# ifpen/wfcrl-env

Hardware: NVIDIA B200
Metric: Floris env-steps/sec (HornsRev1) (higher is better)
Workload: dtype f32

## Files before the change

### wfcrl_b200/csrc/wf_device.cuh

```cuda
#pragma once
#include "../../include/wfcrl_b200.h"

#include <cuda_runtime.h>
#include <stdint.h>

#define WF_MAX_TURBINES_K 128
#define WF_FIX_REC_HDR 5
#define WF_NP 9

struct WfModel {
    int T, B;
    int max_iter, continuous, multi_agent, shaper, table_len;
    int G;
    float yaw_lo_f, yaw_hi_f, yaw_step_f;
    float rate_f, dt_f;
    int autoreset;
    unsigned long long ar_seed;
    long long ar_offset;
    double ar_ti_lo, ar_ti_hi;
    int vtab_tmajor;
    float amb_eps;
    double load_coef, shaper_reference;
    double rho, ref_rho, shear, D, HH, TSR, pP;
    double alpha, beta, ka, kb, ad, bd, dm;
    double ch_const, ch_ai, ch_init, ch_down;
    double e3_112, e3_13;
    const double* layout_c;
    int n_layouts;
    int sample_layouts;
    const double* tab_ws;
    const double* tab_ct;
    const double* tab_pw;
    const double* layout_x;
    const double* layout_y;
};

__host__ __device__ inline const int* layout_counts(const WfModel& m) { return (const int*)(m.layout_c + 2 * m.n_layouts); }

struct WfState {
    double* yaw;
    float* acc;
    float* acc_prev;
    int* num_iter;
    int* num_moves;
    int* nonfinite;
    int* episode;
    uint8_t* amb;
    double* ep_return;
    int* ep_len;
    double* fin_sum;
    double* fin_sumsq;
    int* fin_n;
    long long* fin_len;
    uint8_t* reset_mask;
    int* fix_list;
    int* fix_count;
    double* ws;
    double* wd;
    double* ws_norm;
    double* shaper_ref;
    double* ti_amb;
    double* xs;
    double* ys;
    double* xi;
    double* yi;
    int* order;
    double* cs;
    float2* xhl;
    float2* yhl;
    uchar4* idx;
    double* vtab;
    uint8_t* vtab_ok;
    uint8_t* tab_lo;
    uint8_t* tab_glo;
    double2* vwg;
    int* layout_id;
    int* turbine_count;
};

template <typename R> struct WfFastConstT {
    R ratio[3];
    R mean_ratio;
    R nu4[3];
    R zz[6][3];
    R zz2[6][3];
    R ez[6][3];
    R cblk[48];
    R a_top, a_bot, a_core;
    R inv_ss_den;
    R cv[3][9], cw[3][9];
    R sv[3];
    R D, inv_D, eps2, inv_eps2, inv_2pi;
    R c_top, c_bot, c_wr;
    R alpha4, beta2, ka, kb, ad, bd, dm03, e3_112, e3_13;
    R near_c;
    R d2_8;
    R ch_const, ch_ai, ch_init, ch_down;
    R pP3, rho_fac, ref_rho, two_D, offj[3], dz2[3];
    R load_coef, shaper_reference;
    int table_len;
    R tab_ws[64], tab_ct[64], tab_pw[64];
    unsigned char coarse[128];
    R coarse_scale;
    int coarse_len;
};
typedef WfFastConstT<float> WfFastConst;
typedef WfFastConstT<double> WfFastConst64;

enum WfMode { WF_MODE_INTERFACE = 0, WF_MODE_ENV = 1, WF_MODE_WARMUP = 2 };

struct WfEvalArgs {
    int K;
    int* fix_list;
    int* fix_count;
    uint8_t* amb;
    double2* vwg;
};

cudaError_t wf_launch_geometry(const WfModel& m, const WfState& s, const uint8_t* d_mask, const double* d_cs_override,
                               cudaStream_t stream, bool autoreset_draw = false);
cudaError_t wf_launch_step_basic(int precision, int mode, const WfModel& m, const WfState& s, const uint8_t* d_mask,
                                 const float* d_action, const double* d_yaw_cmd, const WfStepOut& out,
                                 int env_begin, int env_count, cudaStream_t stream);
cudaError_t wf_launch_vortex_table(const WfModel& m, const WfFastConst64& fc, const WfState& s, const uint8_t* d_mask,
                                   cudaStream_t stream);
cudaError_t wf_launch_set_wind(const WfModel& m, const WfState& s, const uint8_t* d_mask, const double* d_ws,
                               const double* d_wd, cudaStream_t stream);
cudaError_t wf_launch_sample_reset(const WfModel& m, const WfState& s, const uint8_t* d_mask, unsigned long long seed,
                                   long long env_id_offset, double ti_lo, double ti_hi, double* d_ws, double* d_wd,
                                   cudaStream_t stream);
cudaError_t wf_launch_reset_state(const WfModel& m, const WfState& s, const uint8_t* d_mask, const double* d_ws,
                                  const double* d_wd, cudaStream_t stream);
cudaError_t wf_step_basic_attributes(int precision, cudaFuncAttributes* attr, int* ctas_per_sm, int threads);
cudaError_t wf_configure_fast_kernels();
cudaError_t wf_configure_fast64_kernels();
cudaError_t wf_launch_step_fast(int mode, bool baked, const WfModel& m, const WfFastConst& fc, const WfState& s,
                                const uint8_t* d_mask, const float* d_action, const double* d_yaw_cmd,
                                const WfStepOut& out, int env_begin, int env_count, cudaStream_t stream);
cudaError_t wf_launch_fixup64(int mode, bool use_vtab, const WfModel& m, const WfFastConst64& fc, const WfState& s,
                              const WfStepOut& out, int env_count, float* d_rec, int rec_cap, cudaStream_t stream);
cudaError_t wf_step_fast_attributes(bool baked, const WfModel& m, cudaFuncAttributes* attr, int* ctas_per_sm, int* threads,
                                    int* smem);
cudaError_t wf_launch_step_fast64(int mode, bool use_vtab, const WfModel& m, const WfFastConst64& fc, const WfState& s,
                                  const uint8_t* d_mask, const float* d_action, const double* d_yaw_cmd,
                                  const WfStepOut& out, int env_begin, int env_count, cudaStream_t stream);
cudaError_t wf_step_fast64_attributes(const WfModel& m, const WfState& s, cudaFuncAttributes* attr, int* ctas_per_sm, int* threads,
                                      int* smem);
cudaError_t wf_launch_eval_fast(bool baked, const WfModel& m, const WfFastConst& fc, const WfState& s, const WfEvalArgs& ev,
                                const double* d_yaw, void* d_power, cudaStream_t stream);
cudaError_t wf_launch_eval_fast64(bool use_vtab, const WfModel& m, const WfFastConst64& fc, const WfState& s,
                                  const WfEvalArgs& ev, const double* d_yaw, void* d_power, cudaStream_t stream);
cudaError_t wf_launch_eval_fixup64(bool use_vtab, const WfModel& m, const WfFastConst64& fc, const WfState& s,
                                   const WfEvalArgs& ev, const double* d_yaw, void* d_power, cudaStream_t stream);
bool wf_fast64_gathers(const WfModel& m, const WfState& s);
```

### wfcrl_b200/csrc/wf_fast.cu

```cuda
#include "wf_device.cuh"
#include "wf_reset_device.cuh"
#include "wf_fast_baked.inc"

namespace {

#define KC(name) (BAKED ? WfBaked::name : fc.name)


constexpr float kLog2e = 1.4426950408889634f;
constexpr float kLn2 = 0.6931471805599453f;
constexpr float kDeg = 57.29577951308232f;
constexpr float kRad = 0.017453292519943295f;
constexpr float kNumEpsF = 0.001f;
constexpr int kTurbPerPass = 10;
constexpr int kMaxEvt = 8;

__device__ __forceinline__ float frcp(float x) { float y; asm("rcp.approx.ftz.f32 %0, %1;" : "=f"(y) : "f"(x)); return y; }
__device__ __forceinline__ float fsqrt(float x) { float y; asm("sqrt.approx.ftz.f32 %0, %1;" : "=f"(y) : "f"(x)); return y; }
__device__ __forceinline__ float fex2(float x) { float y; asm("ex2.approx.ftz.f32 %0, %1;" : "=f"(y) : "f"(x)); return y; }
__device__ __forceinline__ float flg2(float x) { float y; asm("lg2.approx.ftz.f32 %0, %1;" : "=f"(y) : "f"(x)); return y; }
__device__ __forceinline__ float fclamp(float x, float lo, float hi) { return fminf(fmaxf(x, lo), hi); }

__device__ __forceinline__ float interp_f(const WfFastConst& fc, const float* __restrict__ fp, float x, float left,
                                          float right) {
    const int n = fc.table_len;
    const float x0 = fc.tab_ws[0], xn = fc.tab_ws[n - 1];
    if (x < x0) return left;
    if (x > xn) return right;
    int bkt = (int)((x - x0) * fc.coarse_scale);
    bkt = min(bkt, fc.coarse_len - 1);
    int idx = fc.coarse[bkt];
    while (idx + 1 < n - 1 && fc.tab_ws[idx + 1] <= x) ++idx;
    const float xa = fc.tab_ws[idx], fa = fp[idx];
    const float slope = (fp[idx + 1] - fa) * frcp(fc.tab_ws[idx + 1] - xa);
    return fmaf(slope, x - xa, fa);
}

struct SmemView {
    float* wsq;
    float2* vw;
    float2 *xhl, *yhl;
    float *tia;
    float *cyaw, *syaw, *yawr;
    float *tifin;
    float *ynew;
    uchar4* idx;
    unsigned char* ordr;
    unsigned char* queue;
    float4* cblk;
    float* evt_ta;
    uchar2* evt_tj;
};

__host__ __device__ inline size_t fast_smem_bytes(int T) {
    size_t n = 12 * 16;
    n += (size_t)kMaxEvt * 4 + 16;
    n += (size_t)3 * 9 * T * 4;
    n += (size_t)2 * T * 8;
    n += (size_t)3 * T * 4;
    n += (size_t)5 * T * 4;
    n += (size_t)T * 4;
    n += (size_t)((T + 15) / 16 * 16);
    n += (size_t)((T + 15) / 16 * 16);
    return (n + 15) / 16 * 16;
}

__device__ __forceinline__ SmemView carve(unsigned char* base, int T) {
    SmemView s;
    s.cblk = (float4*)base;
    s.evt_ta = (float*)(base + 12 * 16);
    s.evt_tj = (uchar2*)(base + 12 * 16 + kMaxEvt * 4);
    float2* f2 = (float2*)(base + 12 * 16 + kMaxEvt * 4 + 16);
    s.xhl = f2;
    s.yhl = f2 + T;
    s.vw = f2 + 2 * T;
    float* f = (float*)(f2 + 2 * T + 9 * T);
    s.wsq = f; f += 9 * T;
    s.tia = f; f += 3 * T;
    s.cyaw = f; f += T;
    s.syaw = f; f += T;
    s.yawr = f; f += T;
    s.tifin = f; f += T;
    s.ynew = f; f += T;
    s.idx = (uchar4*)f; f += T;
    s.ordr = (unsigned char*)f;
    s.queue = s.ordr + (T + 15) / 16 * 16;
    return s;
}

struct wf_true_tag { static constexpr bool value = true; };
struct wf_false_tag { static constexpr bool value = false; };

template <bool BAKED, bool EVAL = false>
__global__ void __launch_bounds__(32, BAKED ? 16 : 12)
wf_step_fast_kernel(const int mode_, const int env_begin, const WfModel m, const __grid_constant__ WfFastConst fc,
                    const WfState s, const uint8_t* __restrict__ mask, const float* __restrict__ action,
                    const double* __restrict__ yaw_cmd, const WfStepOut out, const WfEvalArgs ev) {
    int b;
    if constexpr (EVAL) b = blockIdx.x / ev.K; else b = blockIdx.x + env_begin;
    const int mode = EVAL ? (int)WF_MODE_INTERFACE : mode_;
    if (mask && !mask[b]) return;
    const int T = m.T;
    const int lane = threadIdx.x;
    const size_t row = (size_t)b * T;
    const size_t orow = EVAL ? (size_t)blockIdx.x * T : row;
    extern __shared__ __align__(16) unsigned char smem_raw[];
    const SmemView sm = carve(smem_raw, T);
    const int n = s.turbine_count[b];

    int nm = 0;
    if (mode == WF_MODE_ENV) nm = s.num_moves[b] + 1;
    for (int tt = lane; tt < n; tt += 32) {
        float ynew;
        if (mode == WF_MODE_ENV) {
            float a = action[row + tt];
            const float acc = s.acc[row + tt];
            const float acc_c = (m.multi_agent && tt != n - 1) ? s.acc_prev[row + tt] : acc;
            const float frac = __fdiv_rn(__fdiv_rn(__fdiv_rn(acc_c, m.rate_f), (float)nm), m.dt_f);
            if (frac >= 0.1f) a = 0.0f;
            if (m.continuous) a = fminf(fmaxf(a, -m.yaw_step_f), m.yaw_step_f);
            else a = __fmul_rn(__fsub_rn(a, 1.0f), m.yaw_step_f);
            const float y0 = fminf(fmaxf((float)s.yaw[row + tt], m.yaw_lo_f), m.yaw_hi_f);
            ynew = fminf(fmaxf(__fadd_rn(y0, a), m.yaw_lo_f), m.yaw_hi_f);
            s.acc_prev[row + tt] = acc;
            s.acc[row + tt] = __fadd_rn(acc, fabsf(a));
            s.yaw[row + tt] = (double)ynew;
        } else if (mode == WF_MODE_INTERFACE && yaw_cmd) {
            const double y = yaw_cmd[orow + tt];
            if (!EVAL) s.yaw[row + tt] = y;
            ynew = (float)y;
        } else {
            ynew = (float)s.yaw[row + tt];
        }
        sm.ynew[tt] = ynew;
        sm.xhl[tt] = s.xhl[row + tt];
        sm.yhl[tt] = s.yhl[row + tt];
        sm.idx[tt] = s.idx[row + tt];
        sm.ordr[tt] = (unsigned char)s.order[row + tt];
    }
    if (lane < 12) sm.cblk[lane] = make_float4(fc.cblk[4 * lane], fc.cblk[4 * lane + 1], fc.cblk[4 * lane + 2], fc.cblk[4 * lane + 3]);
    for (int q = lane; q < 9 * n; q += 32) { sm.wsq[q] = 0.f; sm.vw[q] = make_float2(0.f, 0.f); }
    for (int q = lane; q < 3 * n; q += 32) sm.tia[q] = 0.f;
    __syncwarp();
    for (int tt = lane; tt < n; tt += 32) {
        const float yr = sm.ynew[sm.ordr[tt]] * kRad;
        float sy, cy;
        sincosf(yr, &sy, &cy);
        sm.yawr[tt] = yr;
        sm.cyaw[tt] = cy;
        sm.syaw[tt] = sy;
    }
    const double ws_d = s.ws[b], wd_d = s.wd[b];
    const float ws = (float)ws_d;
    const float I0 = (float)s.ti_amb[b];
    const float I02 = I0 * I0;
    const float I0p = __powf(I0, fc.ch_init);
    const float U0a = ws * fc.ratio[0], U0b = ws * fc.ratio[1], U0c = ws * fc.ratio[2];
    const float D = KC(D);
    __syncwarp();

    const int g = lane / 3, j = lane - 3 * g;
    const bool lane_ok = lane < 3 * kTurbPerPass;
    const float offj = (j == 0) ? fc.offj[0] : ((j == 1) ? fc.offj[1] : fc.offj[2]);
    const int pl = lane & 15;
    const bool pv = pl < 9;
    const int plc = pv ? pl : 0;
    const float U0p = (plc % 3 == 0) ? U0a : ((plc % 3 == 1) ? U0b : U0c);
    const float cvl0 = fc.cv[0][plc], cvl1 = fc.cv[1][plc], cvl2 = fc.cv[2][plc];
    const float cwl0 = fc.cw[0][plc], cwl1 = fc.cw[1][plc], cwl2 = fc.cw[2][plc];
    const float c_dec = KC(eps2) * KC(inv_2pi);
    const float c_e = -KC(inv_eps2) * kLog2e;
    const float c_ek = -(0.5f * kLog2e) * (BAKED ? WfBaked::dz2_0 : fc.dz2[0]);
    const float eps2 = KC(eps2);
    const bool strict = m.amb_eps > 0.f;
    const float thr_lo = 0.05f * (1.f - m.amb_eps), thr_hi = 0.05f * (1.f + m.amb_eps);
    const double two_D_d = 2.0 * m.D;
    int nevt = 0;
    bool flagged = false;

    for (int i = 0; i < n; ++i) {
        float su3, sv, sw, vq, wwq;
        {
            const float wq = sm.wsq[9 * i + plc];
            const float2 vw0 = sm.vw[9 * i + plc];
            vq = vw0.x;
            wwq = vw0.y;
            const float u = U0p - fsqrt(wq);
            su3 = pv ? u * u * u : 0.f;
            sv = pv ? vq : 0.f;
            sw = pv ? wwq : 0.f;
#pragma unroll
            for (int sft = 8; sft > 0; sft >>= 1) {
                su3 += __shfl_xor_sync(0xffffffffu, su3, sft);
                sv += __shfl_xor_sync(0xffffffffu, sv, sft);
                sw += __shfl_xor_sync(0xffffffffu, sw, sft);
            }
        }
        const float avg = cbrtf(su3 * (1.f / 9.f));
        const float ct_raw = fclamp(interp_f(fc, fc.tab_ct, avg, 0.0001f, 0.9999f), 0.0001f, 0.9999f);
        const float cy = sm.cyaw[i], sy = sm.syaw[i], yr = sm.yawr[i];
        const float ct = ct_raw * cy;
        const float s1c = fsqrt(1.f - ct * cy);
        const float a = 0.5f * frcp(cy) * (1.f - s1c);
        const float Gtop0 = KC(c_top) * ws * ct, Gbot0 = KC(c_bot) * ws * ct;
        const float Gwr = KC(c_wr) * (a - a * a) * avg;
        const float Gt = sy * cy * Gtop0, Gb = -(sy * cy * Gbot0);

        float val = 2.f * (sv * (1.f / 9.f) - Gwr * KC(a_core)) * frcp(Gtop0 * KC(a_top) - Gbot0 * KC(a_bot));
        val = fclamp(val, -1.f, 1.f);
        const float g_rad = -(yr + 0.5f * asinf(val));
        const float cg = __cosf(g_rad);

        const float sq1ct = fsqrt(1.f - ct);
        const float sqcg = fsqrt(1.f - ct * cg);
        const float sz0d = 0.5f * D * fsqrt((1.f + sqcg) * frcp(2.f * (1.f + sq1ct)));
        const float sy0d = sz0d * cg;
        const float C0 = 1.f - sq1ct;
        const float M0 = C0 * (2.f - C0);
        const float E0 = C0 * C0 - KC(e3_112) * C0 + KC(e3_13);
        const float th = KC(dm03) * g_rad * frcp(cg) * (1.f - sqcg);
        const float sM0 = fsqrt(M0);
        const float tan_th = __sinf(th) * frcp(__cosf(th));
        const float Kc = th * E0 * (1.f / 5.2f) * fsqrt(sy0d * sz0d * frcp(M0));
        const float A_ln = (1.6f + sM0) * frcp(1.6f - sM0);
        const float inv_s0d = frcp(sy0d * sz0d);

        for (int e = 0; e < min(nevt, kMaxEvt); ++e) {
            const uchar2 tj = sm.evt_tj[e];
            if ((int)tj.x == i && sm.evt_ta[e] > sm.tia[3 * i + tj.y]) flagged = true;
        }
        const float ta0 = sm.tia[3 * i], ta1 = sm.tia[3 * i + 1], ta2 = sm.tia[3 * i + 2];
        const float tp0 = fsqrt(fmaf(ta0, ta0, I02)), tp1 = fsqrt(fmaf(ta1, ta1, I02)), tp2 = fsqrt(fmaf(ta2, ta2, I02));
        const float tpre = (j == 0) ? tp0 : ((j == 1) ? tp1 : tp2);
        const float beta_term = KC(beta2) * (1.f - sq1ct);
        const float x0d = D * cg * (1.f + sqcg) * frcp(1.4142135623730951f * fmaf(KC(alpha4), tpre, beta_term));
        const float kyd = fmaf(KC(ka), tpre, KC(kb));
        const float inv_x0d = frcp(x0d);
        const float delta0 = tan_th * x0d;
        const float Kck = Kc * frcp(kyd);

        const uchar4 ix = sm.idx[i];
        const bool self_on = (int)ix.x <= i;
        float sumV = sv, sumW = sw;
        if (self_on) {
            sumV += Gt * (BAKED ? WfBaked::sv0 : fc.sv[0]) + Gb * (BAKED ? WfBaked::sv1 : fc.sv[1]) +
                    Gwr * (BAKED ? WfBaked::sv2 : fc.sv[2]);
            const float Vs = Gt * cvl0 + Gb * cvl1 + Gwr * cvl2;
            const float Ws = fmaxf(Gt * cwl0 + Gb * cwl1 + Gwr * cwl2, 0.f);
            float rw = pv ? Ws : 0.f;
#pragma unroll
            for (int sft = 8; sft > 0; sft >>= 1) rw += __shfl_xor_sync(0xffffffffu, rw, sft);
            sumW += rw;
            __syncwarp();
            if (lane < 9) sm.vw[9 * i + lane] = make_float2(vq + Vs, wwq + Ws);
        }
        const float aI = avg * tp0;
        const float kk2 = 3.f * aI * aI;
        const float v_term = sumV * (1.f / 9.f), w_term = sumW * (1.f / 9.f);
        const float k_total = 0.5f * (kk2 + v_term * v_term + w_term * w_term);
        const float I_mix = fsqrt((2.f / 3.f) * k_total) * frcp(avg) - tp0;
        const float tq0 = fmaf(2.f, I_mix, tp0), tq1 = fmaf(2.f, I_mix, tp1), tq2 = fmaf(2.f, I_mix, tp2);
        if (lane == 0) sm.tifin[i] = (tq0 + tq1 + tq2) * (1.f / 3.f);
        const float tpost = (j == 0) ? tq0 : ((j == 1) ? tq1 : tq2);

        const float x0v = D * cy * (1.f + sq1ct) * frcp(1.4142135623730951f * fmaf(KC(alpha4), tpost, beta_term));
        const float kyv = fmaf(KC(ka), tpost, KC(kb));
        const float inv_x0v = frcp(x0v);
        const float sz0v = KC(near_c) * (0.5f / 0.501f);
        const float sy0v = sz0v * cy;
        const float near_s = KC(near_c) * fsqrt(ct);
        const float ctc = ct * cy * KC(d2_8);
        const float watK = KC(ch_const) * __powf(a, KC(ch_ai)) * I0p;

        const int lo = ix.x, near_i = ix.y, gt0_i = ix.z, end15 = ix.w;
        const float2 xi = sm.xhl[i], yi = sm.yhl[i];

        constexpr float kCut = 5.5f;
        const float reach1 = kCut * kyv;
        const float reach0 = fmaf(kCut, fmaxf(near_s, sy0v), fabsf(delta0) + fabsf(Kck) * (flg2(A_ln) * kLn2));

        int qn = 0;
        auto v_pass = [&](auto yawed_tag, const int t0) {
            constexpr bool YAWED = decltype(yawed_tag)::value;
            const int tr = t0 + g;
            const bool active = lane_ok && tr < n && tr != i;
            const int t = min(tr, n - 1);
            const float2 xt = sm.xhl[t], yt = sm.yhl[t];
            const float dx = (xt.x - xi.x) + (xt.y - xi.y);
            const float dyc = ((yt.x - yi.x) + (yt.y - yi.y)) + offj;

            const bool need = active && (t >= near_i) &&
                              (fabsf(dyc) < fmaf(reach1, dx, reach0) + fabsf(fmaf(KC(bd), dx, KC(ad))));
            const unsigned nb = __ballot_sync(0xffffffffu, need);
            const bool leader = (j == 0) && active && (((nb >> (3 * g)) & 7u) != 0u);
            const unsigned lb = __ballot_sync(0xffffffffu, leader);
            if (leader) sm.queue[qn + __popc(lb & ((1u << lane) - 1u))] = (unsigned char)t;
            qn += __popc(lb);

            const float yL = dyc + kNumEpsF;
            const float q = yL * yL;
            const float E = fex2(q * c_e);
            float Vk[3], Wk[3];
#pragma unroll
            for (int k = 0; k < 3; ++k) {
                float4 ca, cb, cc, cd;
                if (BAKED) {
                    ca = make_float4(WfBaked::cblk(16 * k), WfBaked::cblk(16 * k + 1), WfBaked::cblk(16 * k + 2), WfBaked::cblk(16 * k + 3));
                    cb = make_float4(WfBaked::cblk(16 * k + 4), WfBaked::cblk(16 * k + 5), WfBaked::cblk(16 * k + 6), WfBaked::cblk(16 * k + 7));
                    cc = make_float4(WfBaked::cblk(16 * k + 8), WfBaked::cblk(16 * k + 9), WfBaked::cblk(16 * k + 10), WfBaked::cblk(16 * k + 11));
                    cd = make_float4(WfBaked::cblk(16 * k + 12), WfBaked::cblk(16 * k + 13), WfBaked::cblk(16 * k + 14), WfBaked::cblk(16 * k + 15));
                } else {
                    ca = sm.cblk[4 * k]; cb = sm.cblk[4 * k + 1]; cc = sm.cblk[4 * k + 2]; cd = sm.cblk[4 * k + 3];
                }
                const float r4 = q + cb.x, r5 = q + cb.y;
                const float g4 = Gwr * frcp(r4 * r5);
                const float X4 = fmaf(-E, cc.x, 1.f) * r5;
                const float NV4 = fmaf(cd.y, X4, -(cd.z * r4));
                float SV, SW;
                if (YAWED) {
                    const float r0 = q + ca.x, r2 = q + ca.y, r1 = q + ca.z, r3 = q + ca.w;
                    const float g0 = Gt * frcp(r0 * r2), g1 = Gb * frcp(r1 * r3);
                    const float X0 = fmaf(-E, cb.z, 1.f) * r2, X1 = fmaf(-E, cb.w, 1.f) * r3;
                    const float NV0 = fmaf(cc.y, X0, -(cc.z * r0)), NV1 = fmaf(cc.w, X1, -(cd.x * r1));
                    SV = fmaf(g4, NV4, fmaf(g1, NV1, g0 * NV0));
                    SW = fmaf(g4, X4 - r4, fmaf(g1, X1 - r1, g0 * (X0 - r0)));
                } else {
                    SV = g4 * NV4;
                    SW = g4 * (X4 - r4);
                }
                const float dec = c_dec * frcp(fmaf(cd.w, dx, eps2));
                Vk[k] = SV * dec;
                Wk[k] = fmaxf(SW * (-yL * dec), 0.f);
            }
            if (active) {
                const int qb = 9 * t + 3 * j;
#pragma unroll
                for (int k = 0; k < 3; ++k) {
                    const float2 o = sm.vw[qb + k];
                    sm.vw[qb + k] = make_float2(o.x + Vk[k], o.y + Wk[k]);
                }
            }
        };
        if (sy != 0.f) {
#pragma unroll 2
            for (int t0 = lo; t0 < n; t0 += kTurbPerPass) v_pass(wf_true_tag{}, t0);
        } else {
#pragma unroll 2
            for (int t0 = lo; t0 < n; t0 += kTurbPerPass) v_pass(wf_false_tag{}, t0);
        }
        __syncwarp();

#pragma unroll 1
        for (int q0 = 0; q0 < qn; q0 += kTurbPerPass) {
            const int e = q0 + g;
            const bool active = lane_ok && e < qn;
            const int t = sm.queue[min(e, qn - 1)];
            const float2 xt = sm.xhl[t], yt = sm.yhl[t];
            const float dx = (xt.x - xi.x) + (xt.y - xi.y);
            const float dyc = ((yt.x - yi.x) + (yt.y - yi.y)) + offj;
            const float lin = fmaf(KC(bd), dx, KC(ad));

            float defl;
            {
                const float dd = dx - x0d;
                const float sgy = fmaf(kyd, dd, sy0d), sgz = fmaf(kyd, dd, sz0d);
                const float sq = fsqrt(sgy * sgz * inv_s0d);
                const float L = flg2(A_ln * fmaf(1.6f, sq, -sM0) * frcp(fmaf(1.6f, sq, sM0))) * kLn2;
                const float d_far = fmaf(Kck, L, delta0) + lin;
                const float d_near = fmaf(dx * inv_x0d, delta0, lin);
                defl = (dx <= x0d) ? d_near : d_far;
            }
            float base, ek;
            {
                const bool far = dx >= x0v;
                const float dd = dx - x0v;
                const float up = dx * inv_x0v, down = 1.f - up;
                const float sgy = far ? fmaf(kyv, dd, sy0v) : fmaf(down, near_s, up * sy0v);
                const float sgz = far ? fmaf(kyv, dd, sz0v) : fmaf(down, near_s, up * sz0v);
                const float ry = frcp(sgy), rz = frcp(sgz);
                const float dy = (dyc - defl) * ry;
                const float dcl = fclamp(fmaf(-ctc * ry, rz, 1.f), 0.f, 1.f);
                const float C = 1.f - fsqrt(dcl);
                base = C * fex2((-0.5f * kLog2e) * dy * dy);
                ek = fex2(c_ek * rz * rz);
            }
            const float be = base * ek;
            const float dU0 = be * U0a, dU1 = base * U0b, dU2 = be * U0c;
            int c = 0;
            if (active) {
                c = ((dU0 > thr_hi) + (dU1 > thr_hi) + (dU2 > thr_hi)) |
                    (((dU0 > thr_lo) + (dU1 > thr_lo) + (dU2 > thr_lo)) << 8);
                const int qb = 9 * t + 3 * j;
                sm.wsq[qb] = fmaf(dU0, dU0, sm.wsq[qb]);
                sm.wsq[qb + 1] = fmaf(dU1, dU1, sm.wsq[qb + 1]);
                sm.wsq[qb + 2] = fmaf(dU2, dU2, sm.wsq[qb + 2]);
            }
            const int gb = 3 * g;
            const int c_tot = __shfl_sync(0xffffffffu, c, gb & 31) + __shfl_sync(0xffffffffu, c, (gb + 1) & 31) +
                              __shfl_sync(0xffffffffu, c, (gb + 2) & 31);
            const int c_lo = c_tot & 0xff, c_hi = c_tot >> 8;
            bool ambiguous = false;
            float ta_hi = 0.f;
            if (active && c_hi > 0 && t >= gt0_i && t < end15) {
                const float ady = fabsf(dyc);
                bool in_win = ady < KC(two_D);
                if (fabsf(ady - KC(two_D)) < 2e-3f) {
                    const double d = (((double)yt.x - (double)yi.x) + ((double)yt.y - (double)yi.y)) + (double)offj;
                    in_win = fabs(d) < two_D_d;
                    if (strict && fabs(fabs(d) - two_D_d) < 1e-7) flagged = true;
                }
                if (in_win) {
                    const float wat = watK * __powf(dx * KC(inv_D), KC(ch_down));
                    if (c_lo > 0) sm.tia[3 * t + j] = fmaxf(sm.tia[3 * t + j], (float)c_lo * (1.f / 9.f) * wat);
                    ambiguous = c_hi != c_lo;
                    ta_hi = (float)c_hi * (1.f / 9.f) * wat;
                }
            }
            const unsigned ab = __ballot_sync(0xffffffffu, ambiguous);
            if (ab) {
                const int slot = nevt + __popc(ab & ((1u << lane) - 1u));
                if (ambiguous) {
                    if (slot < kMaxEvt) { sm.evt_ta[slot] = ta_hi; sm.evt_tj[slot] = make_uchar2((unsigned char)t, (unsigned char)j); }
                    else flagged = true;
                }
                nevt += __popc(ab);
            }
        }
        __syncwarp();
    }

    const bool env = (mode != WF_MODE_INTERFACE);
    const float wd = (float)wd_d;
    float rsum_p = 0.f, rsum_l = 0.f;
    for (int tt = lane; tt < n; tt += 32) {
        float u[9], vv[9], ww[9];
        float su = 0.f, su3 = 0.f, svv = 0.f, sww = 0.f, sdd = 0.f;
#pragma unroll
        for (int p = 0; p < 9; ++p) {
            const float U0k = (p % 3 == 0) ? U0a : ((p % 3 == 1) ? U0b : U0c);
            u[p] = U0k - fsqrt(sm.wsq[9 * tt + p]);
            const float2 vwp = sm.vw[9 * tt + p];
            vv[p] = vwp.x;
            ww[p] = vwp.y;
            su += u[p];
            su3 = fmaf(u[p] * u[p], u[p], su3);
            svv += vv[p];
            sww += ww[p];
            sdd += atan2f(vv[p], u[p]);
        }
        const float avg = cbrtf(su3 * (1.f / 9.f));
        const float mu = su * (1.f / 9.f), mv = svv * (1.f / 9.f), mw = sww * (1.f / 9.f);
        float qu = 0.f, qv = 0.f, qw = 0.f;
#pragma unroll
        for (int p = 0; p < 9; ++p) {
            qu = fmaf(u[p] - mu, u[p] - mu, qu);
            qv = fmaf(vv[p] - mv, vv[p] - mv, qv);
            qw = fmaf(ww[p] - mw, ww[p] - mw, qw);
        }
        const float veff = fc.rho_fac * avg * __powf(sm.cyaw[tt], fc.pP3);
        const float pw = interp_f(fc, fc.tab_pw, veff, 0.f, 0.f) * fc.ref_rho;
        if (strict) {
            constexpr float kVelEps = 1.2e-5f;
            const float pm = interp_f(fc, fc.tab_pw, veff * (1.f - kVelEps), 0.f, 0.f) * fc.ref_rho;
            const float pp = interp_f(fc, fc.tab_pw, veff * (1.f + kVelEps), 0.f, 0.f) * fc.ref_rho;
            if (fmaxf(fabsf(pp - pw), fabsf(pw - pm)) > 1e-4f * fmaxf(pw, 1.f)) flagged = true;
        }
        float wsl = avg;
        float wdl = wd - kDeg * sdd * (1.f / 9.f);
        float loads[4] = {sm.tifin[tt], fsqrt(qu * (1.f / 9.f)), fsqrt(qv * (1.f / 9.f)), fsqrt(qw * (1.f / 9.f))};
        float p_out;
        if (env) {
            p_out = pw * 1e-6f;
            rsum_p += p_out;
            rsum_l += fabsf(loads[0]) + fabsf(loads[1]) + fabsf(loads[2]) + fabsf(loads[3]);
        } else {
            p_out = pw;
#pragma unroll
            for (int q = 0; q < 4; ++q) loads[q] *= 1e7f;
        }
        const int orig = sm.ordr[tt];
        if (EVAL) {
            sm.tifin[tt] = p_out;
            continue;
        }
        float yv = sm.ynew[orig];
        if (mode == WF_MODE_WARMUP) {
            wsl = fclamp(wsl, 3.f, 28.f);
            wdl = fclamp(wdl, 0.f, 360.f);
            yv = fclamp(yv, m.yaw_lo_f, m.yaw_hi_f);
        }
        const size_t o = row + orig;
        if (out.yaw) ((float*)out.yaw)[o] = yv;
        if (out.wind_speed) ((float*)out.wind_speed)[o] = wsl;
        if (out.wind_direction) ((float*)out.wind_direction)[o] = wdl;
        if (out.power) ((float*)out.power)[o] = p_out;
        if (out.load) ((float4*)out.load)[o] = make_float4(loads[0], loads[1], loads[2], loads[3]);
    }
#pragma unroll
    for (int sft = 16; sft > 0; sft >>= 1) {
        rsum_p += __shfl_xor_sync(0xffffffffu, rsum_p, sft);
        rsum_l += __shfl_xor_sync(0xffffffffu, rsum_l, sft);
    }
    const bool any_flag = __any_sync(0xffffffffu, flagged);
    if constexpr (EVAL) {
        if (lane == 0 && ev.amb) ev.amb[blockIdx.x] = (uint8_t)any_flag;
        if (any_flag && strict) {
            if (lane == 0) ev.fix_list[atomicAdd(&ev.fix_count[0], 1)] = blockIdx.x;
            return;
        }
        float* const pw_out = (float*)out.power + orow;
        for (int tt = lane; tt < n; tt += 32) pw_out[sm.ordr[tt]] = sm.tifin[tt];
        for (int tt = n + lane; tt < T; tt += 32) pw_out[tt] = 0.f;
        return;
    }
    if (lane == 0 && s.amb) s.amb[b] = (uint8_t)any_flag;
    if (any_flag && strict) {
        if (lane == 0) s.fix_list[atomicAdd(&s.fix_count[0], 1)] = b;
        return;
    }
    int it = 0;
    if (lane == 0) {
        it = s.num_iter[b] + 1;
        s.num_iter[b] = it;
        if (out.truncated) out.truncated[b] = (uint8_t)(it == m.max_iter);
        float fw0 = ws, fw1 = wd;
        if (mode == WF_MODE_WARMUP) { fw0 = fclamp(fw0, 3.f, 28.f); fw1 = fclamp(fw1, 0.f, 360.f); }
        if (out.freewind) ((float2*)out.freewind)[b] = make_float2(fw0, fw1);
        if (mode == WF_MODE_ENV) {
            s.num_moves[b] = nm;
            const float wn = (float)s.ws_norm[b];
            const float invT = 1.f / (float)n;
            float reward = rsum_p * 1e3f / (wn * wn * wn) * invT - fc.load_coef * rsum_l * (0.25f * invT);
            if (m.shaper == 1) {
                reward = (reward - fc.shaper_reference) / fc.shaper_reference;
            } else if (m.shaper == 2) {
                const double ref = s.shaper_ref[b];
                const float shaped = (ref == 0.0) ? 0.f : (float)(((double)reward - ref) / ref);
                s.shaper_ref[b] = (double)reward;
                reward = shaped;
            }
            if (!isfinite(reward)) s.nonfinite[b] += 1;
            if (out.reward) ((float*)out.reward)[b] = reward;
            wfreset::episode_account(s, b, (double)reward, it == m.max_iter);
            s.ws_norm[b] = ws_d;
        }
    }
    if (mode == WF_MODE_ENV && m.autoreset && __shfl_sync(0xffffffffu, (int)(it == m.max_iter), 0)) {
        for (int tt = lane; tt < T; tt += 32) { s.yaw[row + tt] = 0.0; s.acc[row + tt] = 0.f; s.acc_prev[row + tt] = 0.f; }
        if (lane == 0) wfreset::autoreset_mark(s, b);
    }
    auto zero_padding = [&](void* p, const int w) {
        if (p)
#pragma unroll 1
            for (int q = n * w + lane; q < T * w; q += 32) ((float*)p)[row * w + q] = 0.f;
    };
    zero_padding(out.yaw, 1);
    zero_padding(out.wind_speed, 1);
    zero_padding(out.wind_direction, 1);
    zero_padding(out.power, 1);
    zero_padding(out.load, 4);
}

}

cudaError_t wf_configure_fast_kernels() {
    for (auto k : {wf_step_fast_kernel<true>, wf_step_fast_kernel<false>, wf_step_fast_kernel<true, true>,
                   wf_step_fast_kernel<false, true>}) {
        cudaError_t e = cudaFuncSetAttribute(k, cudaFuncAttributeMaxDynamicSharedMemorySize, 64 * 1024);
        if (e == cudaSuccess)
            e = cudaFuncSetAttribute(k, cudaFuncAttributePreferredSharedMemoryCarveout, cudaSharedmemCarveoutMaxShared);
        if (e != cudaSuccess) return e;
    }
    return cudaSuccess;
}

template <bool BAKED>
static cudaError_t launch_fast_t(int mode, const WfModel& m, const WfFastConst& fc, const WfState& s,
                                 const uint8_t* d_mask, const float* d_action, const double* d_yaw_cmd,
                                 const WfStepOut& out, int env_begin, int env_count, cudaStream_t stream) {
    wf_step_fast_kernel<BAKED><<<env_count, 32, fast_smem_bytes(m.T), stream>>>(mode, env_begin, m, fc, s, d_mask, d_action,
                                                                               d_yaw_cmd, out, WfEvalArgs{});
    return cudaGetLastError();
}

template <bool BAKED>
static cudaError_t launch_eval_t(const WfModel& m, const WfFastConst& fc, const WfState& s, const WfEvalArgs& ev,
                                 const double* d_yaw, void* d_power, cudaStream_t stream) {
    WfStepOut out = {};
    out.power = d_power;
    wf_step_fast_kernel<BAKED, true><<<(unsigned)m.B * (unsigned)ev.K, 32, fast_smem_bytes(m.T), stream>>>(
        WF_MODE_INTERFACE, 0, m, fc, s, nullptr, nullptr, d_yaw, out, ev);
    return cudaGetLastError();
}

cudaError_t wf_launch_eval_fast(bool baked, const WfModel& m, const WfFastConst& fc, const WfState& s, const WfEvalArgs& ev,
                                const double* d_yaw, void* d_power, cudaStream_t stream) {
    return baked ? launch_eval_t<true>(m, fc, s, ev, d_yaw, d_power, stream)
                 : launch_eval_t<false>(m, fc, s, ev, d_yaw, d_power, stream);
}

cudaError_t wf_launch_step_fast(int mode, bool baked, const WfModel& m, const WfFastConst& fc, const WfState& s,
                                const uint8_t* d_mask, const float* d_action, const double* d_yaw_cmd,
                                const WfStepOut& out, int env_begin, int env_count, cudaStream_t stream) {
    return baked ? launch_fast_t<true>(mode, m, fc, s, d_mask, d_action, d_yaw_cmd, out, env_begin, env_count, stream)
                 : launch_fast_t<false>(mode, m, fc, s, d_mask, d_action, d_yaw_cmd, out, env_begin, env_count, stream);
}

template <bool BAKED>
static cudaError_t attrs_fast_t(const WfModel& m, cudaFuncAttributes* attr, int* ctas_per_sm, int* threads, int* smem) {
    *threads = 32;
    *smem = (int)fast_smem_bytes(m.T);
    cudaError_t e = cudaFuncGetAttributes(attr, wf_step_fast_kernel<BAKED>);
    if (e != cudaSuccess) return e;
    return cudaOccupancyMaxActiveBlocksPerMultiprocessor(ctas_per_sm, wf_step_fast_kernel<BAKED>, 32, *smem);
}

cudaError_t wf_step_fast_attributes(bool baked, const WfModel& m, cudaFuncAttributes* attr, int* ctas_per_sm, int* threads,
                                    int* smem) {
    return baked ? attrs_fast_t<true>(m, attr, ctas_per_sm, threads, smem) : attrs_fast_t<false>(m, attr, ctas_per_sm, threads, smem);
}
```

### wfcrl_b200/csrc/wf_host_const.h

```cpp
#pragma once
#include "../../include/wfcrl_b200.h"
#include "wf_device.cuh"

#include <math.h>
#include <string.h>

static inline void wf_fill_default_config(WfConfig* c) {
    memset(c, 0, sizeof(*c));
    c->precision = WF_PREC_F64;
    c->kernel = WF_KERNEL_BASIC;
    c->continuous_control = 1;
    c->reward_shaper = WF_SHAPER_NONE;
    c->yaw_lo = -40.0; c->yaw_hi = 40.0; c->yaw_step = 5.0;
    c->load_coef = 0.1;
    c->shaper_reference = 0.0;
    c->dt = 60.0;
    c->actuator_rate = 0.3;
    c->air_density = 1.225; c->turbulence_intensity = 0.06; c->wind_shear = 0.12; c->wind_veer = 0.0;
    c->alpha = 0.58; c->beta = 0.077; c->ka = 0.38; c->kb = 0.004; c->ad = 0.0; c->bd = 0.0; c->dm = 1.0;
    c->ch_initial = 0.1; c->ch_constant = 0.5; c->ch_ai = 0.8; c->ch_downstream = -0.32;
    c->turbine_grid_points = 3;
    c->rotor_diameter = 126.0; c->hub_height = 90.0; c->tsr = 8.0; c->pP = 1.88; c->pT = 1.88;
    c->generator_efficiency = 1.0; c->ref_density_cp_ct = 1.225;
    static const double cp[51] = {
        0.0, 0.0, 0.0, 0.178085, 0.289075, 0.349022, 0.384728, 0.406059, 0.420228, 0.428823, 0.433873, 0.436223,
        0.436845, 0.436575, 0.436511, 0.436561, 0.436517, 0.435903, 0.434673, 0.433230, 0.430466, 0.378869, 0.335199,
        0.297991, 0.266092, 0.238588, 0.214748, 0.193981, 0.175808, 0.159835, 0.145741, 0.133256, 0.122157, 0.112257,
        0.103399, 0.095449, 0.088294, 0.081836, 0.075993, 0.070692, 0.065875, 0.061484, 0.057476, 0.053809, 0.050447,
        0.047358, 0.044518, 0.041900, 0.039483, 0.0, 0.0};
    static const double ct[51] = {
        0.0, 0.0, 0.0, 0.99, 0.99, 0.97373036, 0.92826162, 0.89210543, 0.86100905, 0.835423, 0.81237673, 0.79225789,
        0.77584769, 0.7629228, 0.76156073, 0.76261984, 0.76169723, 0.75232027, 0.74026851, 0.72987175, 0.70701647,
        0.54054532, 0.45509459, 0.39343381, 0.34250785, 0.30487242, 0.27164979, 0.24361964, 0.21973831, 0.19918151,
        0.18131868, 0.16537679, 0.15103727, 0.13998636, 0.1289037, 0.11970413, 0.11087113, 0.10339901, 0.09617888,
        0.09009926, 0.08395078, 0.0791188, 0.07448356, 0.07050731, 0.06684119, 0.06345518, 0.06032267, 0.05741999,
        0.05472609, 0.0, 0.0};
    c->table_len = 51;
    c->table_ws[0] = 0.0; c->table_ws[1] = 2.0; c->table_ws[2] = 2.5;
    for (int i = 0; i < 45; ++i) c->table_ws[3 + i] = 3.0 + 0.5 * i;
    c->table_ws[48] = 25.01; c->table_ws[49] = 25.02; c->table_ws[50] = 50.0;
    for (int i = 0; i < 51; ++i) { c->table_cp[i] = cp[i]; c->table_ct[i] = ct[i]; }
    }

template <typename R> static inline void build_fast_const(const WfConfig& c, WfFastConstT<R>* f) {
    memset(f, 0, sizeof(*f));
    const double PI = 3.141592653589793, NUM_EPS = 0.001;
    const double D = c.rotor_diameter, HH = c.hub_height, eps = 0.2 * D, eps2 = eps * eps, off = 0.5 * D / 2;
    double Z[3], ratio[3], rsum = 0.0;
    for (int k = 0; k < 3; ++k) {
        Z[k] = HH + (k - 1) * off;
        ratio[k] = pow(Z[k] / HH, c.wind_shear);
        rsum += ratio[k];
    }
    const double mean_ratio = rsum / 3.0;
    f->mean_ratio = (R)mean_ratio;
    const double zc[6] = {-(HH + D / 2), -(HH - D / 2), (HH + D / 2), (HH - D / 2), -HH, HH};
    double zz[6][3];
    for (int k = 0; k < 3; ++k) {
        f->ratio[k] = (R)ratio[k];
        const double dU = c.wind_shear * pow(1.0 / HH, c.wind_shear) * pow(Z[k], c.wind_shear - 1.0);
        const double lmda = D / 8, kappa = 0.41;
        const double lm = kappa * Z[k] / (1 + kappa * Z[k] / lmda);
        f->nu4[k] = (R)(4 * lm * lm * fabs(dU) / mean_ratio);
        for (int q = 0; q < 6; ++q) {
            zz[q][k] = (Z[k] + zc[q]) + NUM_EPS;
            f->zz[q][k] = (R)zz[q][k];
            f->zz2[q][k] = (R)(zz[q][k] * zz[q][k]);
            f->ez[q][k] = (R)exp(-zz[q][k] * zz[q][k] / eps2);
        }
        f->dz2[k] = (R)(((k - 1) * off) * ((k - 1) * off));
        f->offj[k] = (R)((k - 1) * off);
    }
    for (int k = 0; k < 3; ++k) {
        R* c = f->cblk + 16 * k;
        c[0] = f->zz2[0][k]; c[1] = f->zz2[2][k]; c[2] = f->zz2[1][k]; c[3] = f->zz2[3][k];
        c[4] = f->zz2[4][k]; c[5] = f->zz2[5][k]; c[6] = f->ez[0][k]; c[7] = f->ez[1][k];
        c[8] = f->ez[4][k]; c[9] = f->zz[0][k]; c[10] = f->zz[2][k]; c[11] = f->zz[1][k];
        c[12] = f->zz[3][k]; c[13] = f->zz[4][k]; c[14] = f->zz[5][k]; c[15] = f->nu4[k];
    }
    double a_top = 0, a_bot = 0, a_core = 0, sv[3] = {0, 0, 0};
    for (int p = 0; p < 9; ++p) {
        const int j = p / 3, k = p % 3;
        const double yL = (j - 1) * off + NUM_EPS, q = yL * yL;
        double fq[6];
        for (int v = 0; v < 6; ++v) {
            const double r = q + zz[v][k] * zz[v][k];
            fq[v] = (1 - exp(-r / eps2)) / (2 * PI * r);
        }
        a_top += zz[0][k] * fq[0] / 9.0;
        a_bot += zz[1][k] * fq[1] / 9.0;
        a_core += zz[4][k] * fq[4] / 9.0;
        const double cv[3] = {zz[0][k] * fq[0] - zz[2][k] * fq[2], zz[1][k] * fq[1] - zz[3][k] * fq[3],
                              zz[4][k] * fq[4] - zz[5][k] * fq[5]};
        const double cw[3] = {-yL * (fq[0] - fq[2]), -yL * (fq[1] - fq[3]), -yL * (fq[4] - fq[5])};
        for (int v = 0; v < 3; ++v) {
            f->cv[v][p] = (R)cv[v];
            f->cw[v][p] = (R)cw[v];
            sv[v] += cv[v];
        }
    }
    f->a_top = (R)a_top; f->a_bot = (R)a_bot; f->a_core = (R)a_core;
    for (int v = 0; v < 3; ++v) f->sv[v] = (R)sv[v];
    f->D = (R)D; f->inv_D = (R)(1.0 / D); f->eps2 = (R)eps2; f->inv_eps2 = (R)(1.0 / eps2);
    f->inv_2pi = (R)(1.0 / (2 * PI));
    const double vel_top = pow((HH + D / 2) / HH, c.wind_shear), vel_bot = pow((HH - D / 2) / HH, c.wind_shear);
    f->c_top = (R)((PI / 8) * D * vel_top * mean_ratio);
    f->c_bot = (R)((PI / 8) * D * vel_bot * mean_ratio);
    f->c_wr = (R)(0.25 * 2 * PI * D / c.tsr);
    f->inv_ss_den = (R)(1.0 / (((PI / 8) * D * vel_top * mean_ratio) * a_top - ((PI / 8) * D * vel_bot * mean_ratio) * a_bot));
    f->alpha4 = (R)(4 * c.alpha); f->beta2 = (R)(2 * c.beta); f->ka = (R)c.ka; f->kb = (R)c.kb;
    f->ad = (R)c.ad; f->bd = (R)c.bd; f->dm03 = (R)(0.3 * c.dm);
    f->e3_112 = (R)(3 * exp(1.0 / 12.0)); f->e3_13 = (R)(3 * exp(1.0 / 3.0));
    f->near_c = (R)(0.501 * D * sqrt(0.5));
    f->d2_8 = (R)(D * D / 8.0);
    f->ch_const = (R)c.ch_constant; f->ch_ai = (R)c.ch_ai; f->ch_init = (R)c.ch_initial;
    f->ch_down = (R)c.ch_downstream;
    f->pP3 = (R)(c.pP / 3.0); f->rho_fac = (R)cbrt(c.air_density / c.ref_density_cp_ct);
    f->ref_rho = (R)c.ref_density_cp_ct; f->two_D = (R)(2 * D);
    f->load_coef = (R)c.load_coef; f->shaper_reference = (R)c.shaper_reference;
    const int n = c.table_len;
    f->table_len = n;
    const double area = PI * pow(D / 2.0, 2.0);
    for (int i = 0; i < n; ++i) {
        f->tab_ws[i] = (R)c.table_ws[i];
        f->tab_ct[i] = (R)c.table_ct[i];
        f->tab_pw[i] = (R)(0.5 * area * c.table_cp[i] * c.generator_efficiency * pow(c.table_ws[i], 3.0));
    }
    f->coarse_len = 128;
    const double span = c.table_ws[n - 1] - c.table_ws[0];
    f->coarse_scale = (R)(128.0 / span);
    for (int bkt = 0; bkt < 128; ++bkt) {
        const double left = c.table_ws[0] + (bkt - 0.01) * span / 128.0;
        int idx = 0;
        while (idx + 1 < n - 1 && c.table_ws[idx + 1] <= left) ++idx;
        f->coarse[bkt] = (unsigned char)idx;
    }
}
```

Baseline: 5.852 million.

## Precompute table slopes and segment hints; use fast approx pow/cbrt; fold decay constant

Adds precomputed per-segment slopes and a bucket hint table with a multi-node flag to the float fast constants. Table interpolation becomes a single compare plus one FMA, with no division and with the search loop skipped in the common case. cbrtf and __powf are replaced by ex2/lg2-based approximations with one Newton step. The c_dec factor is hoisted out of the inner vortex loop, and lateral-deflection terms are compiled out when the baked ad/bd are zero. The approximations may shift results slightly and the constant struct grows.

```diff
diff --git a/wfcrl_b200/csrc/wf_device.cuh b/wfcrl_b200/csrc/wf_device.cuh
--- a/wfcrl_b200/csrc/wf_device.cuh
+++ b/wfcrl_b200/csrc/wf_device.cuh
@@ -104,7 +104,10 @@
     R coarse_scale;
     int coarse_len;
 };
-typedef WfFastConstT<float> WfFastConst;
+struct WfFastConst : WfFastConstT<float> {
+    float slope_ct[64], slope_pw[64];
+    unsigned char seg[128];
+};
 typedef WfFastConstT<double> WfFastConst64;
 
 enum WfMode { WF_MODE_INTERFACE = 0, WF_MODE_ENV = 1, WF_MODE_WARMUP = 2 };
diff --git a/wfcrl_b200/csrc/wf_fast.cu b/wfcrl_b200/csrc/wf_fast.cu
--- a/wfcrl_b200/csrc/wf_fast.cu
+++ b/wfcrl_b200/csrc/wf_fast.cu
@@ -20,20 +20,26 @@
 __device__ __forceinline__ float fex2(float x) { float y; asm("ex2.approx.ftz.f32 %0, %1;" : "=f"(y) : "f"(x)); return y; }
 __device__ __forceinline__ float flg2(float x) { float y; asm("lg2.approx.ftz.f32 %0, %1;" : "=f"(y) : "f"(x)); return y; }
 __device__ __forceinline__ float fclamp(float x, float lo, float hi) { return fminf(fmaxf(x, lo), hi); }
-
-__device__ __forceinline__ float interp_f(const WfFastConst& fc, const float* __restrict__ fp, float x, float left,
-                                          float right) {
+__device__ __forceinline__ float fpow(float x, float p) { return fex2(p * flg2(x)); }
+__device__ __forceinline__ float fcbrt(float x) {
+    const float ax = fabsf(x);
+    const float y = fex2(flg2(ax) * (1.f / 3.f));
+    const float r = fmaf(fmaf(ax, frcp(y * y), -y), 1.f / 3.f, y);
+    return (ax < 1.17549435e-38f) ? 0.f : copysignf(r, x);
+}
+
+__device__ __forceinline__ float interp_f(const WfFastConst& fc, const float* __restrict__ fp,
+                                          const float* __restrict__ slope, float x, float left, float right) {
     const int n = fc.table_len;
     const float x0 = fc.tab_ws[0], xn = fc.tab_ws[n - 1];
-    if (x < x0) return left;
-    if (x > xn) return right;
-    int bkt = (int)((x - x0) * fc.coarse_scale);
-    bkt = min(bkt, fc.coarse_len - 1);
-    int idx = fc.coarse[bkt];
-    while (idx + 1 < n - 1 && fc.tab_ws[idx + 1] <= x) ++idx;
-    const float xa = fc.tab_ws[idx], fa = fp[idx];
-    const float slope = (fp[idx + 1] - fa) * frcp(fc.tab_ws[idx + 1] - xa);
-    return fmaf(slope, x - xa, fa);
+    const int bkt = min(max((int)((x - x0) * fc.coarse_scale), 0), fc.coarse_len - 1);
+    const int sg = fc.seg[bkt];
+    int idx = sg & 127;
+    if (fc.tab_ws[idx + 1] <= x) ++idx;
+    if (sg >= 128)
+        while (idx + 1 < n - 1 && fc.tab_ws[idx + 1] <= x) ++idx;
+    const float v = fmaf(slope[idx], x - fc.tab_ws[idx], fp[idx]);
+    return (x < x0) ? left : ((x > xn) ? right : v);
 }
 
 struct SmemView {
@@ -154,9 +160,10 @@
     const float ws = (float)ws_d;
     const float I0 = (float)s.ti_amb[b];
     const float I02 = I0 * I0;
-    const float I0p = __powf(I0, fc.ch_init);
+    const float I0p = fpow(I0, fc.ch_init);
     const float U0a = ws * fc.ratio[0], U0b = ws * fc.ratio[1], U0c = ws * fc.ratio[2];
     const float D = KC(D);
+    constexpr bool LIN = !BAKED || WfBaked::ad != 0.f || WfBaked::bd != 0.f;
     __syncwarp();
 
     const int g = lane / 3, j = lane - 3 * g;
@@ -196,8 +203,8 @@
                 sw += __shfl_xor_sync(0xffffffffu, sw, sft);
             }
         }
-        const float avg = cbrtf(su3 * (1.f / 9.f));
-        const float ct_raw = fclamp(interp_f(fc, fc.tab_ct, avg, 0.0001f, 0.9999f), 0.0001f, 0.9999f);
+        const float avg = fcbrt(su3 * (1.f / 9.f));
+        const float ct_raw = fclamp(interp_f(fc, fc.tab_ct, fc.slope_ct, avg, 0.0001f, 0.9999f), 0.0001f, 0.9999f);
         const float cy = sm.cyaw[i], sy = sm.syaw[i], yr = sm.yawr[i];
         const float ct = ct_raw * cy;
         const float s1c = fsqrt(1.f - ct * cy);
@@ -270,7 +277,7 @@
         const float sy0v = sz0v * cy;
         const float near_s = KC(near_c) * fsqrt(ct);
         const float ctc = ct * cy * KC(d2_8);
-        const float watK = KC(ch_const) * __powf(a, KC(ch_ai)) * I0p;
+        const float watK = KC(ch_const) * fpow(a, KC(ch_ai)) * I0p;
 
         const int lo = ix.x, near_i = ix.y, gt0_i = ix.z, end15 = ix.w;
         const float2 xi = sm.xhl[i], yi = sm.yhl[i];
@@ -279,6 +286,7 @@
         const float reach1 = kCut * kyv;
         const float reach0 = fmaf(kCut, fmaxf(near_s, sy0v), fabsf(delta0) + fabsf(Kck) * (flg2(A_ln) * kLn2));
 
+        const float Gt_d = Gt * c_dec, Gb_d = Gb * c_dec, Gwr_d = Gwr * c_dec;
         int qn = 0;
         auto v_pass = [&](auto yawed_tag, const int t0) {
             constexpr bool YAWED = decltype(yawed_tag)::value;
@@ -289,8 +297,9 @@
             const float dx = (xt.x - xi.x) + (xt.y - xi.y);
             const float dyc = ((yt.x - yi.x) + (yt.y - yi.y)) + offj;
 
+            const float reach = fmaf(reach1, dx, reach0);
             const bool need = active && (t >= near_i) &&
-                              (fabsf(dyc) < fmaf(reach1, dx, reach0) + fabsf(fmaf(KC(bd), dx, KC(ad))));
+                              (fabsf(dyc) < (LIN ? reach + fabsf(fmaf(KC(bd), dx, KC(ad))) : reach));
             const unsigned nb = __ballot_sync(0xffffffffu, need);
             const bool leader = (j == 0) && active && (((nb >> (3 * g)) & 7u) != 0u);
             const unsigned lb = __ballot_sync(0xffffffffu, leader);
@@ -313,13 +322,13 @@
                     ca = sm.cblk[4 * k]; cb = sm.cblk[4 * k + 1]; cc = sm.cblk[4 * k + 2]; cd = sm.cblk[4 * k + 3];
                 }
                 const float r4 = q + cb.x, r5 = q + cb.y;
-                const float g4 = Gwr * frcp(r4 * r5);
+                const float g4 = Gwr_d * frcp(r4 * r5);
                 const float X4 = fmaf(-E, cc.x, 1.f) * r5;
                 const float NV4 = fmaf(cd.y, X4, -(cd.z * r4));
                 float SV, SW;
                 if (YAWED) {
                     const float r0 = q + ca.x, r2 = q + ca.y, r1 = q + ca.z, r3 = q + ca.w;
-                    const float g0 = Gt * frcp(r0 * r2), g1 = Gb * frcp(r1 * r3);
+                    const float g0 = Gt_d * frcp(r0 * r2), g1 = Gb_d * frcp(r1 * r3);
                     const float X0 = fmaf(-E, cb.z, 1.f) * r2, X1 = fmaf(-E, cb.w, 1.f) * r3;
                     const float NV0 = fmaf(cc.y, X0, -(cc.z * r0)), NV1 = fmaf(cc.w, X1, -(cd.x * r1));
                     SV = fmaf(g4, NV4, fmaf(g1, NV1, g0 * NV0));
@@ -328,7 +337,7 @@
                     SV = g4 * NV4;
                     SW = g4 * (X4 - r4);
                 }
-                const float dec = c_dec * frcp(fmaf(cd.w, dx, eps2));
+                const float dec = frcp(fmaf(cd.w, dx, eps2));
                 Vk[k] = SV * dec;
                 Wk[k] = fmaxf(SW * (-yL * dec), 0.f);
             }
@@ -366,8 +375,8 @@
                 const float sgy = fmaf(kyd, dd, sy0d), sgz = fmaf(kyd, dd, sz0d);
                 const float sq = fsqrt(sgy * sgz * inv_s0d);
                 const float L = flg2(A_ln * fmaf(1.6f, sq, -sM0) * frcp(fmaf(1.6f, sq, sM0))) * kLn2;
-                const float d_far = fmaf(Kck, L, delta0) + lin;
-                const float d_near = fmaf(dx * inv_x0d, delta0, lin);
+                const float d_far = LIN ? fmaf(Kck, L, delta0) + lin : fmaf(Kck, L, delta0);
+                const float d_near = LIN ? fmaf(dx * inv_x0d, delta0, lin) : dx * inv_x0d * delta0;
                 defl = (dx <= x0d) ? d_near : d_far;
             }
             float base, ek;
@@ -410,7 +419,7 @@
                     if (strict && fabs(fabs(d) - two_D_d) < 1e-7) flagged = true;
                 }
                 if (in_win) {
-                    const float wat = watK * __powf(dx * KC(inv_D), KC(ch_down));
+                    const float wat = watK * fpow(dx * KC(inv_D), KC(ch_down));
                     if (c_lo > 0) sm.tia[3 * t + j] = fmaxf(sm.tia[3 * t + j], (float)c_lo * (1.f / 9.f) * wat);
                     ambiguous = c_hi != c_lo;
                     ta_hi = (float)c_hi * (1.f / 9.f) * wat;
@@ -448,7 +457,7 @@
             sww += ww[p];
             sdd += atan2f(vv[p], u[p]);
         }
-        const float avg = cbrtf(su3 * (1.f / 9.f));
+        const float avg = fcbrt(su3 * (1.f / 9.f));
         const float mu = su * (1.f / 9.f), mv = svv * (1.f / 9.f), mw = sww * (1.f / 9.f);
         float qu = 0.f, qv = 0.f, qw = 0.f;
 #pragma unroll
@@ -457,12 +466,12 @@
             qv = fmaf(vv[p] - mv, vv[p] - mv, qv);
             qw = fmaf(ww[p] - mw, ww[p] - mw, qw);
         }
-        const float veff = fc.rho_fac * avg * __powf(sm.cyaw[tt], fc.pP3);
-        const float pw = interp_f(fc, fc.tab_pw, veff, 0.f, 0.f) * fc.ref_rho;
+        const float veff = fc.rho_fac * avg * fpow(sm.cyaw[tt], fc.pP3);
+        const float pw = interp_f(fc, fc.tab_pw, fc.slope_pw, veff, 0.f, 0.f) * fc.ref_rho;
         if (strict) {
             constexpr float kVelEps = 1.2e-5f;
-            const float pm = interp_f(fc, fc.tab_pw, veff * (1.f - kVelEps), 0.f, 0.f) * fc.ref_rho;
-            const float pp = interp_f(fc, fc.tab_pw, veff * (1.f + kVelEps), 0.f, 0.f) * fc.ref_rho;
+            const float pm = interp_f(fc, fc.tab_pw, fc.slope_pw, veff * (1.f - kVelEps), 0.f, 0.f) * fc.ref_rho;
+            const float pp = interp_f(fc, fc.tab_pw, fc.slope_pw, veff * (1.f + kVelEps), 0.f, 0.f) * fc.ref_rho;
             if (fmaxf(fabsf(pp - pw), fabsf(pw - pm)) > 1e-4f * fmaxf(pw, 1.f)) flagged = true;
         }
         float wsl = avg;
diff --git a/wfcrl_b200/csrc/wf_host_const.h b/wfcrl_b200/csrc/wf_host_const.h
--- a/wfcrl_b200/csrc/wf_host_const.h
+++ b/wfcrl_b200/csrc/wf_host_const.h
@@ -41,6 +41,11 @@
     c->table_ws[48] = 25.01; c->table_ws[49] = 25.02; c->table_ws[50] = 50.0;
     for (int i = 0; i < 51; ++i) { c->table_cp[i] = cp[i]; c->table_ct[i] = ct[i]; }
     }
+
+static inline double wf_table_power(const WfConfig& c, int i) {
+    const double PI = 3.141592653589793;
+    return 0.5 * (PI * pow(c.rotor_diameter / 2.0, 2.0)) * c.table_cp[i] * c.generator_efficiency * pow(c.table_ws[i], 3.0);
+}
 
 template <typename R> static inline void build_fast_const(const WfConfig& c, WfFastConstT<R>* f) {
     memset(f, 0, sizeof(*f));
@@ -120,11 +125,10 @@
     f->load_coef = (R)c.load_coef; f->shaper_reference = (R)c.shaper_reference;
     const int n = c.table_len;
     f->table_len = n;
-    const double area = PI * pow(D / 2.0, 2.0);
     for (int i = 0; i < n; ++i) {
         f->tab_ws[i] = (R)c.table_ws[i];
         f->tab_ct[i] = (R)c.table_ct[i];
-        f->tab_pw[i] = (R)(0.5 * area * c.table_cp[i] * c.generator_efficiency * pow(c.table_ws[i], 3.0));
+        f->tab_pw[i] = (R)wf_table_power(c, i);
     }
     f->coarse_len = 128;
     const double span = c.table_ws[n - 1] - c.table_ws[0];
@@ -136,3 +140,22 @@
         f->coarse[bkt] = (unsigned char)idx;
     }
 }
+
+static inline void build_fast_const(const WfConfig& c, WfFastConst* f) {
+    build_fast_const<float>(c, f);
+    memset(f->slope_ct, 0, sizeof(f->slope_ct));
+    memset(f->slope_pw, 0, sizeof(f->slope_pw));
+    const int n = c.table_len;
+    for (int k = 0; k + 1 < n; ++k) {
+        const double dws = c.table_ws[k + 1] - c.table_ws[k];
+        f->slope_ct[k] = (float)((c.table_ct[k + 1] - c.table_ct[k]) / dws);
+        f->slope_pw[k] = (float)((wf_table_power(c, k + 1) - wf_table_power(c, k)) / dws);
+    }
+    const double span = c.table_ws[n - 1] - c.table_ws[0];
+    for (int bkt = 0; bkt < 128; ++bkt) {
+        const double left = c.table_ws[0] + (bkt - 0.01) * span / 128.0, right = c.table_ws[0] + (bkt + 1.01) * span / 128.0;
+        int nodes = 0;
+        for (int k = 1; k < n - 1; ++k) nodes += (c.table_ws[k] > left && c.table_ws[k] <= right);
+        f->seg[bkt] = (unsigned char)(f->coarse[bkt] + (nodes > 1 ? 128 : 0));
+    }
+}
```

Result: faster. 6.026 million (median of 6 runs) (+3.0%).
